# Jittor/PointCloudLib

Measured on AMD Instinct MI355X. Metric: point-clouds/sec fwd+bwd, PointNet++ SSG B=32 N=1024, higher is better.
Workload: dtype f32; 1 GPU; PointNet++ SSG cls train step (fwd+bwd+SGD), B=32/GPU, N=1024 xyz+normal, gauss_ball clouds (BASELINE configs[1]); global_batch=32, n_points=1024, parallelism=dp1, launch=eager, grad_overlap=False, cpu_affinity=numa node 1 (gpu0), 128 cpus, world_size=1, sync_bn=False, entry_points=per-stack (pcl_mlp_stack_*_f32)

## Files before the change

### pointcloudlib_amd/csrc/compact.hip

```cpp
#include "common.h"

namespace pcl {

struct GoffMulti { const int32_t* cnt[4]; int32_t* goff[4]; };
__device__ __forceinline__ void group_offsets_body(const int32_t* __restrict__ cnt, int G, int32_t* __restrict__ goff);
__global__ __launch_bounds__(1024) void group_offsets_kernel(const int32_t* __restrict__ cnt, int G, int32_t* __restrict__ goff) {
    group_offsets_body(cnt, G, goff);
}
__global__ __launch_bounds__(1024) void group_offsets_multi_kernel(const GoffMulti a, int G) {
    group_offsets_body(a.cnt[blockIdx.x], G, a.goff[blockIdx.x]);
}
__device__ __forceinline__ void group_offsets_body(const int32_t* __restrict__ cnt, int G, int32_t* __restrict__ goff) {
    __shared__ int tot[16];
    constexpr int U = 8;
    const int lane = threadIdx.x & 63, w = threadIdx.x >> 6;
    const int per = ((G + 15) / 16 + 63) / 64 * 64;
    const int lo = min(w * per, G), hi = min(lo + per, G);
    int s = 0;
    rows_in_flight<U>(cnt, 1, lo + lane, 64, hi, [&](int, int v) { s += max(v, 1); });
#pragma unroll
    for (int o = 32; o > 0; o >>= 1) s += __shfl_xor(s, o);
    if (lane == 0) tot[w] = s;
    __syncthreads();
    int run = 0, all = 0;
// ... 198 lines not shown
                                                           const int32_t* __restrict__ n_rows, int C1, float* __restrict__ Y,
                                                           double* __restrict__ stats) {
    __shared__ double red[2][4][64 * NH];
    const int wave = threadIdx.x >> 6, lane = threadIdx.x & 63;
    const int R = *n_rows;
    float wx[NH][3], wf[NH][GL_CF];
    double ss[NH], qq[NH];
#pragma unroll
    for (int h = 0; h < NH; ++h) {
        const int ch = lane + 64 * h;
#pragma unroll
        for (int d = 0; d < 3; ++d) wx[h][d] = (Wx && ch < C1) ? Wx[(size_t)ch * ldw + d] : 0.f;
#pragma unroll
        for (int f = 0; f < GL_CF; ++f) wf[h][f] = (f < CF && ch < C1) ? Wfs[(size_t)ch * ldw + f] : 0.f;
        ss[h] = 0.0; qq[h] = 0.0;
    }
    const int stride = gridDim.x * 4 * GL_RPI;
    int r0 = (blockIdx.x * 4 + wave) * GL_RPI;
    float4 nl[GL_RPI], nf[GL_RPI]; int sr[GL_RPI];
#pragma unroll
    for (int j = 0; j < GL_RPI; ++j) {
        const int r = min(r0 + j, R - 1);
        nl[j] = rloc[r]; sr[j] = Uf ? rsrc[r] : 0; nf[j] = CF ? rfeat[r] : make_float4(0.f, 0.f, 0.f, 0.f);
    }
    for (; r0 < R; r0 += stride) {
        float4 L[GL_RPI], F[GL_RPI]; int cs[GL_RPI];
#pragma unroll
        for (int j = 0; j < GL_RPI; ++j) { L[j] = nl[j]; F[j] = nf[j]; cs[j] = sr[j]; }
        {
            const int rn = r0 + stride;
#pragma unroll
            for (int j = 0; j < GL_RPI; ++j) {
                const int r = min(rn + j, R - 1);
                nl[j] = rloc[r]; sr[j] = Uf ? rsrc[r] : 0; nf[j] = CF ? rfeat[r] : make_float4(0.f, 0.f, 0.f, 0.f);
            }
        }
#pragma unroll
        for (int h = 0; h < NH; ++h) {
            const int ch = min(lane + 64 * h, C1 - 1);
            float u[GL_RPI];
#pragma unroll
            for (int j = 0; j < GL_RPI; ++j) u[j] = Uf ? Uf[(size_t)cs[j] * C1 + ch] : 0.f;
#pragma unroll
            for (int j = 0; j < GL_RPI; ++j) {
                if (r0 + j < R && lane + 64 * h < C1) {
                    const float y = glin_row_value(u[j], L[j], F[j], wx[h], wf[h]);
                    Y[(size_t)(r0 + j) * C1 + ch] = y;
                    const double w = (double)L[j].w;
                    ss[h] += w * (double)y; qq[h] += w * (double)y * (double)y;
                }
            }
        }
    }
#pragma unroll
    for (int h = 0; h < NH; ++h) { red[0][wave][lane + 64 * h] = ss[h]; red[1][wave][lane + 64 * h] = qq[h]; }
    __syncthreads();
    for (int ch = threadIdx.x; ch < C1; ch += 256) {
        double* dst = stats + (size_t)blockIdx.x * 2 * C1;
        dst[ch] = (red[0][0][ch] + red[0][1][ch]) + (red[0][2][ch] + red[0][3][ch]);
        dst[C1 + ch] = (red[1][0][ch] + red[1][1][ch]) + (red[1][2][ch] + red[1][3][ch]);
    }
}

template <int NH>
__global__ __launch_bounds__(256) void group_linear_bwd_kernel(const float4* __restrict__ rloc, const float4* __restrict__ rfeat,
                                                               int CF, const float* __restrict__ dU, const float* __restrict__ Y,
                                                               const float* __restrict__ a_, const float* __restrict__ k1_,
                                                               const float* __restrict__ k2_, const float* __restrict__ mu_,
                                                               const int32_t* __restrict__ rsrc,
                                                               const int32_t* __restrict__ n_rows, int C1, float* __restrict__ dUf,
                                                               float* __restrict__ dWx_part, float* __restrict__ dWf_part) {
    __shared__ float red[3 + GL_CF][4][64 * NH];
    const int wave = threadIdx.x >> 6, lane = threadIdx.x & 63;
    const int R = *n_rows;
    float a[NH], k1[NH], k2[NH], mu[NH], gw[NH][3 + GL_CF];
#pragma unroll
    for (int h = 0; h < NH; ++h) {
        const int ch = min(lane + 64 * h, C1 - 1);
        a[h] = a_[ch]; k1[h] = k1_[ch]; k2[h] = k2_[ch]; mu[h] = mu_[ch];
#pragma unroll
        for (int d = 0; d < 3 + GL_CF; ++d) gw[h][d] = 0.f;
    }
    const int stride = gridDim.x * 4 * GL_RPI;
    int r0 = (blockIdx.x * 4 + wave) * GL_RPI;
    float4 nl[GL_RPI], nf[GL_RPI]; int sr[GL_RPI];
#pragma unroll
    for (int j = 0; j < GL_RPI; ++j) {
        const int r = min(r0 + j, R - 1);
        nl[j] = rloc[r]; sr[j] = dUf ? rsrc[r] : 0; nf[j] = dWf_part ? rfeat[r] : make_float4(0.f, 0.f, 0.f, 0.f);
    }
    for (; r0 < R; r0 += stride) {
        float4 L[GL_RPI], F[GL_RPI]; int cs[GL_RPI];
#pragma unroll
        for (int j = 0; j < GL_RPI; ++j) { L[j] = nl[j]; F[j] = nf[j]; cs[j] = sr[j]; }
        {
            const int rn = r0 + stride;
#pragma unroll
            for (int j = 0; j < GL_RPI; ++j) {
                const int r = min(rn + j, R - 1);
                nl[j] = rloc[r]; sr[j] = dUf ? rsrc[r] : 0; nf[j] = dWf_part ? rfeat[r] : make_float4(0.f, 0.f, 0.f, 0.f);
            }
        }
#pragma unroll
        for (int h = 0; h < NH; ++h) {
            const int ch = min(lane + 64 * h, C1 - 1);
            float du[GL_RPI], y[GL_RPI];
#pragma unroll
            for (int j = 0; j < GL_RPI; ++j) {
                const size_t o = (size_t)min(r0 + j, R - 1) * C1 + ch;
                du[j] = dU[o]; y[j] = Y[o];
            }
#pragma unroll
            for (int j = 0; j < GL_RPI; ++j) {
                if (r0 + j < R && lane + 64 * h < C1) {
                    const float dy = fmaf(a[h], du[j], -L[j].w * fmaf(k2[h], y[j] - mu[h], k1[h]));
                    if (dUf) unsafeAtomicAdd(&dUf[(size_t)cs[j] * C1 + ch], dy);
                    gw[h][0] = fmaf(dy, L[j].x, gw[h][0]); gw[h][1] = fmaf(dy, L[j].y, gw[h][1]);
                    gw[h][2] = fmaf(dy, L[j].z, gw[h][2]);
                    gw[h][3] = fmaf(dy, F[j].x, gw[h][3]); gw[h][4] = fmaf(dy, F[j].y, gw[h][4]);
                    gw[h][5] = fmaf(dy, F[j].z, gw[h][5]); gw[h][6] = fmaf(dy, F[j].w, gw[h][6]);
                }
            }
        }
    }
    if (dWx_part || dWf_part) {
#pragma unroll
        for (int h = 0; h < NH; ++h)
#pragma unroll
            for (int d = 0; d < 3 + GL_CF; ++d) red[d][wave][lane + 64 * h] = gw[h][d];
        __syncthreads();
        if (dWx_part)
            for (int e = threadIdx.x; e < C1 * 3; e += 256) {
                const int ch = e / 3, d = e - ch * 3;
                dWx_part[(size_t)blockIdx.x * C1 * 3 + e] = (red[d][0][ch] + red[d][1][ch]) + (red[d][2][ch] + red[d][3][ch]);
            }
        if (dWf_part)
            for (int e = threadIdx.x; e < C1 * CF; e += 256) {
                const int ch = e / CF, d = 3 + (e - ch * CF);
                dWf_part[(size_t)blockIdx.x * C1 * CF + e] = (red[d][0][ch] + red[d][1][ch]) + (red[d][2][ch] + red[d][3][ch]);
            }
    }
}

__device__ __forceinline__ void glin_load_weights(const float* __restrict__ Wx, const float* __restrict__ Wfs, int CF, int ldw, int c4,
                                                  float (&wx)[4][3], float (&wf)[4][GL_CF]) {
#pragma unroll
    for (int v = 0; v < 4; ++v) {
#pragma unroll
        for (int d = 0; d < 3; ++d) wx[v][d] = Wx ? Wx[(size_t)(c4 + v) * ldw + d] : 0.f;
#pragma unroll
        for (int f = 0; f < GL_CF; ++f) wf[v][f] = f < CF ? Wfs[(size_t)(c4 + v) * ldw + f] : 0.f;
    }
}
template <int LPR>
__global__ __launch_bounds__(256) void group_linear_v4_kernel(const float* __restrict__ Uf, const float* __restrict__ Wx,
                                                              const float* __restrict__ Wfs, int CF, int ldw,
                                                              const float4* __restrict__ rloc, const float4* __restrict__ rfeat,
                                                              const int32_t* __restrict__ rsrc,
                                                              const int32_t* __restrict__ n_rows, float* __restrict__ Y,
                                                              double* __restrict__ stats) {
    constexpr int C1 = 4 * LPR, RPW = 64 / LPR, U = 4;
    __shared__ double red[2][4][C1];
    const int wave = threadIdx.x >> 6, lane = threadIdx.x & 63;
    const int cl = lane % LPR, rsub = lane / LPR, c4 = 4 * cl;
    const int R = *n_rows;
    float wx[4][3], wf[4][GL_CF];
    double ss[4], qq[4];
#pragma unroll
    for (int v = 0; v < 4; ++v) {
#pragma unroll
        for (int d = 0; d < 3; ++d) wx[v][d] = Wx ? Wx[(size_t)(c4 + v) * ldw + d] : 0.f;
#pragma unroll
        for (int f = 0; f < GL_CF; ++f) wf[v][f] = f < CF ? Wfs[(size_t)(c4 + v) * ldw + f] : 0.f;
        ss[v] = 0.0; qq[v] = 0.0;
    }
    const int stride = gridDim.x * 4 * RPW * U;
    for (int r0 = (blockIdx.x * 4 + wave) * RPW * U; r0 < R; r0 += stride) {
        float4 L[U], F[U], u[U];
#pragma unroll
        for (int j = 0; j < U; ++j) {
            const int r = min(r0 + j * RPW + rsub, R - 1);
            L[j] = rloc[r];
            F[j] = CF ? rfeat[r] : make_float4(0.f, 0.f, 0.f, 0.f);
            u[j] = Uf ? *reinterpret_cast<const float4*>(Uf + (size_t)rsrc[r] * C1 + c4) : make_float4(0.f, 0.f, 0.f, 0.f);
        }
#pragma unroll
        for (int j = 0; j < U; ++j) {
            const int r = r0 + j * RPW + rsub;
            if (r < R) {
                float y[4] = {u[j].x, u[j].y, u[j].z, u[j].w};
                const double w = (double)L[j].w;
#pragma unroll
                for (int v = 0; v < 4; ++v) {
                    const float t = glin_row_value(y[v], L[j], F[j], wx[v], wf[v]);
                    y[v] = t;
                    ss[v] += w * (double)t; qq[v] += w * (double)t * (double)t;
                }
                *reinterpret_cast<float4*>(Y + (size_t)r * C1 + c4) = make_float4(y[0], y[1], y[2], y[3]);
            }
        }
    }
#pragma unroll
    for (int v = 0; v < 4; ++v) {
#pragma unroll
        for (int off = LPR; off < 64; off <<= 1) { ss[v] += __shfl_xor(ss[v], off); qq[v] += __shfl_xor(qq[v], off); }
        if (rsub == 0) { red[0][wave][c4 + v] = ss[v]; red[1][wave][c4 + v] = qq[v]; }
    }
    __syncthreads();
    for (int ch = threadIdx.x; ch < C1; ch += 256) {
        double* dst = stats + (size_t)blockIdx.x * 2 * C1;
        dst[ch] = (red[0][0][ch] + red[0][1][ch]) + (red[0][2][ch] + red[0][3][ch]);
        dst[C1 + ch] = (red[1][0][ch] + red[1][1][ch]) + (red[1][2][ch] + red[1][3][ch]);
    }
}

template <int LPR>
__global__ __launch_bounds__(256) void group_linear_bwd_v4_kernel(const float4* __restrict__ rloc, const float4* __restrict__ rfeat,
                                                                  int CF, const float* __restrict__ dU, const float* __restrict__ Y,
                                                                  const float* __restrict__ a_, const float* __restrict__ k1_,
                                                                  const float* __restrict__ k2_, const float* __restrict__ mu_,
                                                                  const int32_t* __restrict__ rsrc,
                                                                  const int32_t* __restrict__ n_rows, float* __restrict__ dUf,
                                                                  float* __restrict__ dWx_part, float* __restrict__ dWf_part) {
    constexpr int C1 = 4 * LPR, RPW = 64 / LPR, U = 4;
    __shared__ float red[3 + GL_CF][4][C1];
    const int wave = threadIdx.x >> 6, lane = threadIdx.x & 63;
    const int cl = lane % LPR, rsub = lane / LPR, c4 = 4 * cl;
    const int R = *n_rows;
    float a[4], k1[4], k2[4], mu[4], gw[3 + GL_CF][4];
#pragma unroll
    for (int v = 0; v < 4; ++v) {
        a[v] = a_[c4 + v]; k1[v] = k1_[c4 + v]; k2[v] = k2_[c4 + v]; mu[v] = mu_[c4 + v];
#pragma unroll
        for (int d = 0; d < 3 + GL_CF; ++d) gw[d][v] = 0.f;
    }
    const int stride = gridDim.x * 4 * RPW * U;
    for (int r0 = (blockIdx.x * 4 + wave) * RPW * U; r0 < R; r0 += stride) {
        float4 L[U], F[U], du[U], yv[U];
        int src[U];
#pragma unroll
        for (int j = 0; j < U; ++j) {
            const int r = min(r0 + j * RPW + rsub, R - 1);
            L[j] = rloc[r];
            F[j] = dWf_part ? rfeat[r] : make_float4(0.f, 0.f, 0.f, 0.f);
            src[j] = dUf ? rsrc[r] : 0;
            du[j] = *reinterpret_cast<const float4*>(dU + (size_t)r * C1 + c4);
            yv[j] = *reinterpret_cast<const float4*>(Y + (size_t)r * C1 + c4);
        }
#pragma unroll
        for (int j = 0; j < U; ++j) {
            const int r = r0 + j * RPW + rsub;
            if (r < R) {
                const float dd[4] = {du[j].x, du[j].y, du[j].z, du[j].w}, yy[4] = {yv[j].x, yv[j].y, yv[j].z, yv[j].w};
#pragma unroll
                for (int v = 0; v < 4; ++v) {
                    const float dy = fmaf(a[v], dd[v], -L[j].w * fmaf(k2[v], yy[v] - mu[v], k1[v]));
                    if (dUf) unsafeAtomicAdd(&dUf[(size_t)src[j] * C1 + c4 + v], dy);
                    gw[0][v] = fmaf(dy, L[j].x, gw[0][v]); gw[1][v] = fmaf(dy, L[j].y, gw[1][v]); gw[2][v] = fmaf(dy, L[j].z, gw[2][v]);
                    gw[3][v] = fmaf(dy, F[j].x, gw[3][v]); gw[4][v] = fmaf(dy, F[j].y, gw[4][v]);
                    gw[5][v] = fmaf(dy, F[j].z, gw[5][v]); gw[6][v] = fmaf(dy, F[j].w, gw[6][v]);
                }
            }
        }
    }
    if (dWx_part || dWf_part) {
#pragma unroll
        for (int d = 0; d < 3 + GL_CF; ++d)
#pragma unroll
            for (int v = 0; v < 4; ++v) {
                float t = gw[d][v];
#pragma unroll
                for (int off = LPR; off < 64; off <<= 1) t += __shfl_xor(t, off);
                if (rsub == 0) red[d][wave][c4 + v] = t;
            }
        __syncthreads();
        if (dWx_part)
            for (int e = threadIdx.x; e < C1 * 3; e += 256) {
                const int ch = e / 3, d = e - ch * 3;
                dWx_part[(size_t)blockIdx.x * C1 * 3 + e] = (red[d][0][ch] + red[d][1][ch]) + (red[d][2][ch] + red[d][3][ch]);
            }
        if (dWf_part)
            for (int e = threadIdx.x; e < C1 * CF; e += 256) {
                const int ch = e / CF, d = 3 + (e - ch * CF);
                dWf_part[(size_t)blockIdx.x * C1 * CF + e] = (red[d][0][ch] + red[d][1][ch]) + (red[d][2][ch] + red[d][3][ch]);
            }
    }
}

template <int LPR>
__global__ __launch_bounds__(256) void group_linear_bwd_regen_kernel(const float4* __restrict__ rloc, const float4* __restrict__ rfeat,
                                                                     const float* __restrict__ Wx, const float* __restrict__ Wfs, int CF,
                                                                     int ldw, const float* __restrict__ dU, const float* __restrict__ a_,
                                                                     const float* __restrict__ k1_, const float* __restrict__ k2_,
                                                                     const float* __restrict__ mu_, const int32_t* __restrict__ n_rows,
                                                                     float* __restrict__ dWx_part, float* __restrict__ dWf_part) {
    constexpr int C1 = 4 * LPR, RPW = 64 / LPR, CH = 4, U = 3;
    __shared__ float red[3 + GL_CF][4][C1];
    const int wave = threadIdx.x >> 6, lane = threadIdx.x & 63;
    const int cl = lane % LPR, rsub = lane / LPR, c4 = 4 * cl;
    const int R = *n_rows;
    float wx[4][3], wf[4][GL_CF];
    float a[4], k1[4], k2[4], mu[4], gw[3 + GL_CF][4];
    glin_load_weights(Wx, Wfs, CF, ldw, c4, wx, wf);
#pragma unroll
    for (int v = 0; v < 4; ++v) {
        a[v] = a_[c4 + v]; k1[v] = k1_[c4 + v]; k2[v] = k2_[c4 + v]; mu[v] = mu_[c4 + v];
#pragma unroll
        for (int d = 0; d < 3 + GL_CF; ++d) gw[d][v] = 0.f;
    }
    const int stride = gridDim.x * 4 * RPW * CH, base = (blockIdx.x * 4 + wave) * RPW * CH;
    for (int t0 = 0; base + (t0 / CH) * stride < R; t0 += U) {
        float4 L[U], F[U], du[U];
        int row[U];
#pragma unroll
        for (int j = 0; j < U; ++j) {
            const int t = t0 + j;
            row[j] = base + (t / CH) * stride + (t % CH) * RPW + rsub;
            const int r = min(row[j], R - 1);
            L[j] = rloc[r];
            F[j] = CF ? rfeat[r] : make_float4(0.f, 0.f, 0.f, 0.f);
            du[j] = *reinterpret_cast<const float4*>(dU + (size_t)r * C1 + c4);
        }
#pragma unroll
        for (int j = 0; j < U; ++j) {
            if (row[j] < R) {
                const float dd[4] = {du[j].x, du[j].y, du[j].z, du[j].w};
#pragma unroll
                for (int v = 0; v < 4; ++v) {
                    const float y = glin_row_value(0.f, L[j], F[j], wx[v], wf[v]);
                    const float dy = fmaf(a[v], dd[v], -L[j].w * fmaf(k2[v], y - mu[v], k1[v]));
                    gw[0][v] = fmaf(dy, L[j].x, gw[0][v]); gw[1][v] = fmaf(dy, L[j].y, gw[1][v]); gw[2][v] = fmaf(dy, L[j].z, gw[2][v]);
                    gw[3][v] = fmaf(dy, F[j].x, gw[3][v]); gw[4][v] = fmaf(dy, F[j].y, gw[4][v]);
                    gw[5][v] = fmaf(dy, F[j].z, gw[5][v]); gw[6][v] = fmaf(dy, F[j].w, gw[6][v]);
                }
            }
        }
    }
#pragma unroll
    for (int d = 0; d < 3 + GL_CF; ++d)
#pragma unroll
        for (int v = 0; v < 4; ++v) {
            float t = gw[d][v];
#pragma unroll
            for (int off = LPR; off < 64; off <<= 1) t += __shfl_xor(t, off);
            if (rsub == 0) red[d][wave][c4 + v] = t;
        }
    __syncthreads();
    if (dWx_part)
        for (int e = threadIdx.x; e < C1 * 3; e += 256) {
            const int ch = e / 3, d = e - ch * 3;
            dWx_part[(size_t)blockIdx.x * C1 * 3 + e] = (red[d][0][ch] + red[d][1][ch]) + (red[d][2][ch] + red[d][3][ch]);
        }
// ... 192 lines not shown
    __syncthreads();
    int run = inc - s;
    for (int w = 0; w < wave; ++w) run += wtot[w];
    for (int i = i0; i < i1; ++i) {
        const int t = off[i];
        off[i] = run;
        int pos = run;
        for (int w = 0; w < RT_W; ++w) { const int c = cnt[w * N + i]; cnt[w * N + i] = pos; pos += c; }
        run += t;
    }
    if (tid == 0) off[N] = re - rb;
    __syncthreads();
    for (int g = g0; g < g1; ++g) {
        const int q0 = group_off[g_first + g], q1 = group_off[g_first + g + 1];
        for (int r = q0 + lane; r < q1; r += 64) lst[atomicAdd(&mycnt[rsrc[r] - pbase], 1)] = r;
        __builtin_amdgcn_fence(__ATOMIC_SEQ_CST, "wavefront");
        __builtin_amdgcn_wave_barrier();
    }
    __syncthreads();
    for (int pl = tid; pl < N; pl += RT_T) in_off[pbase + pl] = rb + off[pl];
    if (b == B - 1 && tid == 0) in_off[pbase + N] = re;
    for (int i = tid; i < re - rb; i += RT_T) in_rows[rb + i] = lst[i];
}

__global__ __launch_bounds__(256) void group_linear_dw_kernel(const float* __restrict__ px, const float* __restrict__ pf, int rows,
                                                              int C1, int CF, int off, int ld, float* __restrict__ dW0) {
    const int nx = px ? C1 * 3 : 0, nf = pf ? C1 * CF : 0;
    const int e = blockIdx.x * 4 + (threadIdx.x >> 6), lane = threadIdx.x & 63;
    if (e >= nx + nf) return;
    const bool isx = e < nx;
    const float* src = isx ? px + e : pf + (e - nx);
    const int n = isx ? nx : nf;
    float s = 0.f;
    rows_in_flight<8>(src, n, lane, 64, rows, [&](int, float v) { s += v; });
#pragma unroll
    for (int o = 32; o > 0; o >>= 1) s += __shfl_xor(s, o);
    if (lane == 0) {
        if (isx) dW0[(size_t)(e / 3) * ld + e % 3] = s;
        else dW0[(size_t)((e - nx) / CF) * ld + off + (e - nx) % CF] = s;
    }
}

}
using namespace pcl;

extern "C" int pcl_group_offsets_i32(const int32_t* cnt, int G, int32_t* group_off, void* stream) {
    PCL_REQUIRE(cnt && group_off && G >= 1, "pcl_group_offsets_i32: bad arguments");
    hipLaunchKernelGGL(group_offsets_kernel, dim3(1), dim3(1024), 0, as_stream(stream), cnt, G, group_off);
    return check_launch("pcl_group_offsets_i32");
}

extern "C" int pcl_group_offsets_multi_i32(int n, const int32_t* const* cnt, int G, int32_t* const* group_off, void* stream) {
    PCL_REQUIRE(cnt && group_off && G >= 1 && n >= 1 && n <= 4, "pcl_group_offsets_multi_i32: bad arguments (n = %d: 1..4)", n);
    GoffMulti a = {};
    for (int i = 0; i < n; ++i) {
        PCL_REQUIRE(cnt[i] && group_off[i], "pcl_group_offsets_multi_i32: null array %d", i);
        a.cnt[i] = cnt[i]; a.goff[i] = group_off[i];
    }
    hipLaunchKernelGGL(group_offsets_multi_kernel, dim3(n), dim3(1024), 0, as_stream(stream), a, G);
    return check_launch("pcl_group_offsets_multi_i32");
}

extern "C" int pcl_group_compact_f32(const float* xyz, const float* new_xyz, const float* feat, const int32_t* idx,
                                     const int32_t* cnt, const int32_t* group_off, int B, int N, int m, int ns, int C,
                                     int use_xyz, int row_stride, float* rows, int32_t* row_meta, int32_t* row_src,
                                     void* stream) {
    PCL_REQUIRE(idx && cnt && rows && row_meta && row_src && group_off, "pcl_group_compact_f32: null pointer");
    PCL_REQUIRE(!use_xyz || (xyz && new_xyz), "pcl_group_compact_f32: use_xyz needs xyz and new_xyz");
    PCL_REQUIRE(C == 0 || feat, "pcl_group_compact_f32: C=%d needs feat", C);
    PCL_REQUIRE(B >= 1 && N >= 1 && m >= 1 && ns >= 1 && ns < 32768 && C >= 0 && (use_xyz || C > 0), "pcl_group_compact_f32: bad sizes");
    const int D = (use_xyz ? 3 : 0) + C;
    PCL_REQUIRE(row_stride >= D && row_stride < D + 64, "pcl_group_compact_f32: row_stride=%d for %d columns", row_stride, D);
    const int G = B * m;
    hipLaunchKernelGGL(group_compact_kernel, dim3(G), dim3(256), 0, as_stream(stream), xyz, new_xyz, feat, idx, cnt, group_off, G, N, m,
                       ns, C, use_xyz, row_stride, rows, reinterpret_cast<int2*>(row_meta), row_src);
    return check_launch("pcl_group_compact_f32");
}

extern "C" int pcl_bn_act_max_rows_f32(const float* Y, const int32_t* group_off, const float* scale, const float* shift,
                                       float slope, int G, int C, float* out, int32_t* arg, float* ymax, void* stream) {
    PCL_REQUIRE(Y && group_off && scale && shift && out && arg && ymax && G >= 1 && C >= 1, "pcl_bn_act_max_rows_f32: bad arguments");
    const bool vec = (C % 4 == 0) && al16(Y);
    const size_t total = (size_t)G * (vec ? C / 4 : C);
    int blocks = (int)((total + 255) / 256);
    if (blocks > 16384) blocks = 16384;
    if (vec)
        hipLaunchKernelGGL(bn_act_max_rows_kernel<4>, dim3(blocks), dim3(256), 0, as_stream(stream), Y, group_off, scale, shift, slope,
                           G, C, out, arg, ymax);
    else
        hipLaunchKernelGGL(bn_act_max_rows_kernel<1>, dim3(blocks), dim3(256), 0, as_stream(stream), Y, group_off, scale, shift, slope,
                           G, C, out, arg, ymax);
    return check_launch("pcl_bn_act_max_rows_f32");
}

extern "C" int pcl_scatter_rows_add_f32(const float* grows, const int32_t* row_src, const int32_t* n_rows_dev, int rows_cap,
                                        int D, int off, int C, int n_dst_rows, float* gfeat, void* stream) {
    PCL_REQUIRE(grows && row_src && n_rows_dev && gfeat && rows_cap >= 1 && D >= 1 && off >= 0 && C >= 1 && off + C <= D && n_dst_rows >= 1,
                "pcl_scatter_rows_add_f32: bad arguments");
    hipStream_t st = as_stream(stream);
    hipError_t e = hipMemsetAsync(gfeat, 0, sizeof(float) * (size_t)n_dst_rows * C, st);
    if (e != hipSuccess) return fail(PCL_EHIP, "pcl_scatter_rows_add_f32: memset: %s", hipGetErrorString(e));
    size_t blocks = ((size_t)rows_cap + 7) / 8;
    if (blocks > 8192) blocks = 8192;
    hipLaunchKernelGGL(scatter_rows_add_kernel, dim3((int)blocks), dim3(256), 0, st, grows, row_src, n_rows_dev, D, off, C, gfeat);
    return check_launch("pcl_scatter_rows_add_f32");
}

constexpr int GL_BLOCKS = 1024;

extern "C" int pcl_group_linear_stat_rows(int B, int m) { return (B < 1 || m < 1) ? 0 : GL_BLOCKS; }

namespace pcl {
int group_linear_fwd_impl(const float* xyz, const float* new_xyz, const float* Uf, const float* Wx, const float* feat_small,
                          const float* Wf_small, int CF, int ldw, const int32_t* idx, const int32_t* cnt, const int32_t* group_off, int B,
                          int N, int m, int ns, int C1, float* Y, int32_t* row_meta, int32_t* row_src, float* row_loc, float* row_feat,
                          double* stats_ws, void* stream, int phase, const float* dense_src, float* dense_dst, int dense_cols);
}
extern "C" int pcl_group_linear_f32(const float* xyz, const float* new_xyz, const float* Uf, const float* Wx, const float* feat_small,
                                    const float* Wf_small, int CF, int ldw, const int32_t* idx, const int32_t* cnt,
                                    const int32_t* group_off, int B, int N, int m, int ns, int C1, float* Y, int32_t* row_meta,
                                    int32_t* row_src, float* row_loc, float* row_feat, double* stats_ws, void* stream) {
    return group_linear_fwd_impl(xyz, new_xyz, Uf, Wx, feat_small, Wf_small, CF, ldw, idx, cnt, group_off, B, N, m, ns, C1, Y, row_meta, row_src,
                                 row_loc, row_feat, stats_ws, stream, 3, nullptr, nullptr, 0);
}
int pcl::group_linear_fwd_impl(const float* xyz, const float* new_xyz, const float* Uf, const float* Wx, const float* feat_small,
                               const float* Wf_small, int CF, int ldw, const int32_t* idx, const int32_t* cnt, const int32_t* group_off,
                               int B, int N, int m, int ns, int C1, float* Y, int32_t* row_meta, int32_t* row_src, float* row_loc,
                               float* row_feat, double* stats_ws, void* stream, int phase, const float* dense_src, float* dense_dst,
                               int dense_cols) {
    PCL_REQUIRE(idx && cnt && group_off && Y && row_meta && row_src && row_loc && stats_ws, "pcl_group_linear_f32: null pointer");
    PCL_REQUIRE(CF == 0 || row_feat, "pcl_group_linear_f32: inline features need row_feat");
    PCL_REQUIRE(phase == 1 || Uf || Wx || CF > 0, "pcl_group_linear_f32: need features (Uf or feat_small) and/or coordinates (Wx)");
    PCL_REQUIRE(CF >= 0 && CF <= GL_CF && (CF == 0 || (feat_small && Wf_small)), "pcl_group_linear_f32: CF=%d inline features (<= %d)", CF, GL_CF);
    PCL_REQUIRE(!Wx || (xyz && new_xyz), "pcl_group_linear_f32: Wx needs xyz and new_xyz");
    PCL_REQUIRE(ldw >= (Wx ? 3 : 0) && ldw >= CF, "pcl_group_linear_f32: ldw=%d", ldw);
    PCL_REQUIRE(B >= 1 && N >= 1 && m >= 1 && ns >= 1 && ns < 32768 && C1 >= 1 && C1 <= 64 * GL_MAXH,
                "pcl_group_linear_f32: bad sizes B=%d N=%d m=%d ns=%d C1=%d (C1 <= %d)", B, N, m, ns, C1, 64 * GL_MAXH);
    const int G = B * m;
    hipStream_t st = as_stream(stream);
    if (phase & 1) {
        const int gb = (G + 3) / 4;
        DenseJob dj = {dense_src, dense_dst, C1, dense_cols, ldw, gb, 0};
        if (dense_dst) dj.blocks = (C1 * dense_cols + 1023) / 1024 < 64 ? (C1 * dense_cols + 1023) / 1024 : 64;
        hipLaunchKernelGGL(group_rows_meta_kernel, dim3(gb + dj.blocks), dim3(256), 0, st, Wx ? xyz : nullptr, new_xyz, feat_small, CF, idx, cnt,
                           group_off, G, N, m, ns, reinterpret_cast<int2*>(row_meta), row_src, reinterpret_cast<float4*>(row_loc),
                           reinterpret_cast<float4*>(CF ? row_feat : nullptr), dj);
        int rc = check_launch("pcl_group_linear_f32(meta)");
        if (rc || phase == 1) return rc;
    }
    const float4* rl = reinterpret_cast<const float4*>(row_loc);
    const float4* rf = reinterpret_cast<const float4*>(row_feat);
    const dim3 grid(GL_BLOCKS), block(256);
    if (al16(Y, Uf) && (C1 == 64 || C1 == 128 || C1 == 256)) {
        if (C1 == 64) hipLaunchKernelGGL(group_linear_v4_kernel<16>, grid, block, 0, st, Uf, Wx, Wf_small, CF, ldw, rl, rf, row_src, group_off + G, Y, stats_ws);
        else if (C1 == 128) hipLaunchKernelGGL(group_linear_v4_kernel<32>, grid, block, 0, st, Uf, Wx, Wf_small, CF, ldw, rl, rf, row_src, group_off + G, Y, stats_ws);
        else hipLaunchKernelGGL(group_linear_v4_kernel<64>, grid, block, 0, st, Uf, Wx, Wf_small, CF, ldw, rl, rf, row_src, group_off + G, Y, stats_ws);
        return check_launch("pcl_group_linear_f32");
    }
    if (C1 <= 64) hipLaunchKernelGGL(group_linear_kernel<1>, grid, block, 0, st, Uf, Wx, Wf_small, CF, ldw, rl, rf, row_src, group_off + G, C1, Y, stats_ws);
    else if (C1 <= 128) hipLaunchKernelGGL(group_linear_kernel<2>, grid, block, 0, st, Uf, Wx, Wf_small, CF, ldw, rl, rf, row_src, group_off + G, C1, Y, stats_ws);
    else hipLaunchKernelGGL(group_linear_kernel<4>, grid, block, 0, st, Uf, Wx, Wf_small, CF, ldw, rl, rf, row_src, group_off + G, C1, Y, stats_ws);
    return check_launch("pcl_group_linear_f32");
}

namespace pcl {
int group_linear_bwd_impl(const float* row_loc, const float* row_feat, int CF, const float* dU, const float* Y, const float* a,
                          const float* k1, const float* k2, const float* mu, const int32_t* row_src, const int32_t* n_rows_dev, int B, int N,
                          int C1, float* dUf, float* dWx_part, float* dWf_part, float* dW0, int ldw, int off, void* stream, bool duf_is_zero);
}
extern "C" int pcl_group_linear_bwd_f32(const float* row_loc, const float* row_feat, int CF, const float* dU, const float* Y,
                                        const float* a, const float* k1, const float* k2, const float* mu, const int32_t* row_src,
                                        const int32_t* n_rows_dev, int B, int N, int C1, float* dUf, float* dWx_part,
                                        float* dWf_part, float* dW0, int ldw, int off, void* stream) {
    return group_linear_bwd_impl(row_loc, row_feat, CF, dU, Y, a, k1, k2, mu, row_src, n_rows_dev, B, N, C1, dUf, dWx_part, dWf_part, dW0, ldw,
                                 off, stream, false);
}
int pcl::group_linear_bwd_impl(const float* row_loc, const float* row_feat, int CF, const float* dU, const float* Y, const float* a,
                               const float* k1, const float* k2, const float* mu, const int32_t* row_src, const int32_t* n_rows_dev, int B,
                               int N, int C1, float* dUf, float* dWx_part, float* dWf_part, float* dW0, int ldw, int off, void* stream,
                               bool duf_is_zero) {
    PCL_REQUIRE(row_loc && dU && Y && a && k1 && k2 && mu && row_src && n_rows_dev, "pcl_group_linear_bwd_f32: null pointer");
    PCL_REQUIRE(dUf || dWx_part || dWf_part, "pcl_group_linear_bwd_f32: nothing to compute");
    PCL_REQUIRE(!dWf_part || (row_feat && CF >= 1 && CF <= GL_CF), "pcl_group_linear_bwd_f32: dWf needs row_feat, CF=%d", CF);
    PCL_REQUIRE(B >= 1 && N >= 1 && C1 >= 1 && C1 <= 64 * GL_MAXH, "pcl_group_linear_bwd_f32: bad sizes");
    PCL_REQUIRE(!dW0 || ((dWx_part || dWf_part) && ldw >= (dWx_part ? 3 : 0) && off >= 0 && ldw >= off + (dWf_part ? CF : 0)),
                "pcl_group_linear_bwd_f32: dW0 needs the partial buffers and ldw=%d >= off=%d + CF", ldw, off);
    hipStream_t st = as_stream(stream);
    if (dUf && !duf_is_zero) {
        hipError_t e = hipMemsetAsync(dUf, 0, sizeof(float) * (size_t)B * N * C1, st);
        if (e != hipSuccess) return fail(PCL_EHIP, "pcl_group_linear_bwd_f32: memset: %s", hipGetErrorString(e));
    }
    const float4* rl = reinterpret_cast<const float4*>(row_loc);
    const float4* rf = reinterpret_cast<const float4*>(row_feat);
    const dim3 grid(GL_BLOCKS), block(256);
    if (!dUf && al16(Y, dU) && (C1 == 64 || C1 == 128 || C1 == 256)) {
        if (C1 == 64) hipLaunchKernelGGL(group_linear_bwd_v4_kernel<16>, grid, block, 0, st, rl, rf, CF, dU, Y, a, k1, k2, mu, row_src, n_rows_dev, dUf, dWx_part, dWf_part);
        else if (C1 == 128) hipLaunchKernelGGL(group_linear_bwd_v4_kernel<32>, grid, block, 0, st, rl, rf, CF, dU, Y, a, k1, k2, mu, row_src, n_rows_dev, dUf, dWx_part, dWf_part);
        else hipLaunchKernelGGL(group_linear_bwd_v4_kernel<64>, grid, block, 0, st, rl, rf, CF, dU, Y, a, k1, k2, mu, row_src, n_rows_dev, dUf, dWx_part, dWf_part);
    } else if (C1 <= 64) hipLaunchKernelGGL(group_linear_bwd_kernel<1>, grid, block, 0, st, rl, rf, CF, dU, Y, a, k1, k2, mu, row_src, n_rows_dev, C1, dUf, dWx_part, dWf_part);
    else if (C1 <= 128) hipLaunchKernelGGL(group_linear_bwd_kernel<2>, grid, block, 0, st, rl, rf, CF, dU, Y, a, k1, k2, mu, row_src, n_rows_dev, C1, dUf, dWx_part, dWf_part);
    else hipLaunchKernelGGL(group_linear_bwd_kernel<4>, grid, block, 0, st, rl, rf, CF, dU, Y, a, k1, k2, mu, row_src, n_rows_dev, C1, dUf, dWx_part, dWf_part);
    int rc = check_launch("pcl_group_linear_bwd_f32");
    if (rc || !dW0) return rc;
    const int n = (dWx_part ? C1 * 3 : 0) + (dWf_part ? C1 * CF : 0);
    hipLaunchKernelGGL(group_linear_dw_kernel, dim3((n + 3) / 4), block, 0, st, dWx_part, dWf_part, GL_BLOCKS, C1, CF, off, ldw, dW0);
    return check_launch("pcl_group_linear_bwd_f32(dW)");
}

extern "C" int pcl_group_linear_dw_sum_f32(const float* dWx_part, const float* dWf_part, int rows, int C1, int CF, int off, int ld, float* dW0,
                                           void* stream) {
    PCL_REQUIRE((dWx_part || dWf_part) && dW0 && rows >= 1 && C1 >= 1, "pcl_group_linear_dw_sum_f32: bad arguments");
    PCL_REQUIRE(!dWf_part || CF >= 1, "pcl_group_linear_dw_sum_f32: dWf_part needs CF >= 1");
    PCL_REQUIRE(ld >= (dWx_part ? 3 : 0) && off >= 0 && ld >= off + (dWf_part ? CF : 0), "pcl_group_linear_dw_sum_f32: ld=%d below off=%d + CF", ld, off);
    const int n = (dWx_part ? C1 * 3 : 0) + (dWf_part ? C1 * CF : 0);
    hipLaunchKernelGGL(group_linear_dw_kernel, dim3((n + 3) / 4), dim3(256), 0, as_stream(stream), dWx_part, dWf_part, rows, C1, CF, off, ld, dW0);
    return check_launch("pcl_group_linear_dw_sum_f32");
}

extern "C" int pcl_group_rows_transpose_supported(int N, int m, int ns) {
    return N >= 1 && m >= 1 && ns >= 1 && ((size_t)(RT_W + 1) * N + 1 + (size_t)m * ns) * 4 <= 150 * 1024;
}
extern "C" int pcl_group_rows_transpose_i32(const int32_t* row_src, const int32_t* group_off, int B, int N, int m, int ns, int32_t* in_off,
                                            int32_t* in_rows, void* stream) {
    PCL_REQUIRE(row_src && group_off && in_off && in_rows && B >= 1 && m >= 1 && ns >= 1, "pcl_group_rows_transpose_i32: bad arguments");
    PCL_REQUIRE(pcl_group_rows_transpose_supported(N, m, ns), "pcl_group_rows_transpose_i32: N=%d m=%d ns=%d beyond the LDS-resident form", N, m, ns);
    const size_t lds = ((size_t)(RT_W + 1) * N + 1 + (size_t)m * ns) * 4;
    auto kern = rows_transpose_kernel;
    if (int rc = lds_opt_in(kern, lds, "pcl_group_rows_transpose_i32")) return rc;
    hipLaunchKernelGGL(kern, dim3(B), dim3(RT_T), lds, as_stream(stream), row_src, group_off, m, N, B, in_off, in_rows);
    return check_launch("pcl_group_rows_transpose_i32");
}
extern "C" int pcl_group_linear_bwd_gather_supported(int C1) { return g_lab.scatter_gather && (C1 == 64 || C1 == 128 || C1 == 256); }
extern "C" int pcl_group_linear_bwd_gather_f32(const float* row_loc, const float* dU, const float* Y, const float* a, const float* k1,
                                               const float* k2, const float* mu, const int32_t* in_off, const int32_t* in_rows, int B, int N,
                                               int C1, float* dUf, float* dWx_part, float* dW0, int ldw, void* stream) {
    PCL_REQUIRE(row_loc && dU && Y && a && k1 && k2 && mu && in_off && in_rows && dUf, "pcl_group_linear_bwd_gather_f32: null pointer");
    PCL_REQUIRE(B >= 1 && N >= 1 && pcl_group_linear_bwd_gather_supported(C1), "pcl_group_linear_bwd_gather_f32: bad sizes (C1 = %d: 64, 128 or 256)", C1);
    PCL_REQUIRE(al16(dU, Y, dUf) && al16(a, k1, k2, mu), "pcl_group_linear_bwd_gather_f32: 16-byte aligned rows");
    PCL_REQUIRE(!dW0 || (dWx_part && ldw >= 3), "pcl_group_linear_bwd_gather_f32: dW0 needs dWx_part and ldw >= 3");
    hipStream_t st = as_stream(stream);
    const float4* rl = reinterpret_cast<const float4*>(row_loc);
    const dim3 grid(GL_BLOCKS), block(256);
    const int P = B * N;
    if (C1 == 64) hipLaunchKernelGGL(group_linear_bwd_gather_kernel<16>, grid, block, 0, st, rl, dU, Y, a, k1, k2, mu, in_off, in_rows, P, dUf, dWx_part);
    else if (C1 == 128) hipLaunchKernelGGL(group_linear_bwd_gather_kernel<32>, grid, block, 0, st, rl, dU, Y, a, k1, k2, mu, in_off, in_rows, P, dUf, dWx_part);
    else hipLaunchKernelGGL(group_linear_bwd_gather_kernel<64>, grid, block, 0, st, rl, dU, Y, a, k1, k2, mu, in_off, in_rows, P, dUf, dWx_part);
    int rc = check_launch("pcl_group_linear_bwd_gather_f32");
    if (rc || !dW0) return rc;
    hipLaunchKernelGGL(group_linear_dw_kernel, dim3((C1 * 3 + 3) / 4), block, 0, st, dWx_part, (const float*)nullptr, GL_BLOCKS, C1, 0, 0, ldw, dW0);
    return check_launch("pcl_group_linear_bwd_gather_f32(dW)");
}

extern "C" int pcl_group_linear_bwd_regen_supported(int C1, int CF) {
    return (C1 == 64 || C1 == 128 || C1 == 256) && CF >= 0 && CF <= GL_CF;
}
extern "C" int pcl_group_linear_bwd_regen_f32(const float* row_loc, const float* row_feat, const float* Wx, const float* Wf_small, int CF,
                                              int ldw, const float* dU, const float* a, const float* k1, const float* k2, const float* mu,
                                              const int32_t* n_rows_dev, int C1, float* dWx_part, float* dWf_part, float* dW0, int ld0, int off,
                                              void* stream) {
    PCL_REQUIRE(row_loc && dU && a && k1 && k2 && mu && n_rows_dev, "pcl_group_linear_bwd_regen_f32: null pointer");
    PCL_REQUIRE(pcl_group_linear_bwd_regen_supported(C1, CF), "pcl_group_linear_bwd_regen_f32: C1 = %d (64, 128 or 256), CF = %d (<= %d)", C1, CF, GL_CF);
    PCL_REQUIRE(Wx || CF > 0, "pcl_group_linear_bwd_regen_f32: need the forward's weights (Wx and/or Wf_small)");
    PCL_REQUIRE(CF == 0 || (row_feat && Wf_small), "pcl_group_linear_bwd_regen_f32: CF=%d inline features need row_feat and Wf_small", CF);
    PCL_REQUIRE(ldw >= (Wx ? 3 : 0) && ldw >= CF, "pcl_group_linear_bwd_regen_f32: ldw=%d", ldw);
    PCL_REQUIRE(dWx_part || dWf_part, "pcl_group_linear_bwd_regen_f32: nothing to compute");
    PCL_REQUIRE(!dWf_part || CF >= 1, "pcl_group_linear_bwd_regen_f32: dWf_part needs CF >= 1");
    PCL_REQUIRE(al16(dU, row_loc, row_feat), "pcl_group_linear_bwd_regen_f32: 16-byte aligned rows");
    PCL_REQUIRE(!dW0 || (ld0 >= (dWx_part ? 3 : 0) && off >= 0 && ld0 >= off + (dWf_part ? CF : 0)),
                "pcl_group_linear_bwd_regen_f32: dW0 needs ld0=%d >= off=%d + CF", ld0, off);
    hipStream_t st = as_stream(stream);
    const float4* rl = reinterpret_cast<const float4*>(row_loc);
    const float4* rf = reinterpret_cast<const float4*>(row_feat);
    const dim3 grid(GL_BLOCKS), block(256);
    if (C1 == 64) hipLaunchKernelGGL(group_linear_bwd_regen_kernel<16>, grid, block, 0, st, rl, rf, Wx, Wf_small, CF, ldw, dU, a, k1, k2, mu, n_rows_dev, dWx_part, dWf_part);
    else if (C1 == 128) hipLaunchKernelGGL(group_linear_bwd_regen_kernel<32>, grid, block, 0, st, rl, rf, Wx, Wf_small, CF, ldw, dU, a, k1, k2, mu, n_rows_dev, dWx_part, dWf_part);
    else hipLaunchKernelGGL(group_linear_bwd_regen_kernel<64>, grid, block, 0, st, rl, rf, Wx, Wf_small, CF, ldw, dU, a, k1, k2, mu, n_rows_dev, dWx_part, dWf_part);
    int rc = check_launch("pcl_group_linear_bwd_regen_f32");
    if (rc || !dW0) return rc;
    const int n = (dWx_part ? C1 * 3 : 0) + (dWf_part ? C1 * CF : 0);
    hipLaunchKernelGGL(group_linear_dw_kernel, dim3((n + 3) / 4), block, 0, st, dWx_part, dWf_part, GL_BLOCKS, C1, CF, off, ld0, dW0);
    return check_launch("pcl_group_linear_bwd_regen_f32(dW)");
}
extern "C" int pcl_group_linear_bwd_gather_regen_f32(const float* row_loc, const float* dU, const float* Uf, const float* Wx, int ldw,
                                                     const float* a, const float* k1, const float* k2, const float* mu, const int32_t* in_off,
                                                     const int32_t* in_rows, int B, int N, int C1, float* dUf, float* dWx_part, float* dW0,
                                                     int ld0, void* stream) {
    PCL_REQUIRE(row_loc && dU && Uf && a && k1 && k2 && mu && in_off && in_rows && dUf, "pcl_group_linear_bwd_gather_regen_f32: null pointer");
    PCL_REQUIRE(B >= 1 && N >= 1 && pcl_group_linear_bwd_gather_supported(C1), "pcl_group_linear_bwd_gather_regen_f32: bad sizes (C1 = %d: 64, 128 or 256)", C1);
    PCL_REQUIRE(al16(dU, Uf, dUf, row_loc) && al16(a, k1, k2, mu), "pcl_group_linear_bwd_gather_regen_f32: 16-byte aligned rows");
    PCL_REQUIRE(!Wx || ldw >= 3, "pcl_group_linear_bwd_gather_regen_f32: ldw=%d", ldw);
    PCL_REQUIRE(!dW0 || (dWx_part && ld0 >= 3), "pcl_group_linear_bwd_gather_regen_f32: dW0 needs dWx_part and ld0 >= 3");
    hipStream_t st = as_stream(stream);
    const float4* rl = reinterpret_cast<const float4*>(row_loc);
    const dim3 grid(GL_BLOCKS), block(256);
    const int P = B * N;
    if (C1 == 64) hipLaunchKernelGGL(group_linear_bwd_gather_regen_kernel<16>, grid, block, 0, st, rl, dU, Uf, Wx, ldw, a, k1, k2, mu, in_off, in_rows, P, dUf, dWx_part);
    else if (C1 == 128) hipLaunchKernelGGL(group_linear_bwd_gather_regen_kernel<32>, grid, block, 0, st, rl, dU, Uf, Wx, ldw, a, k1, k2, mu, in_off, in_rows, P, dUf, dWx_part);
    else hipLaunchKernelGGL(group_linear_bwd_gather_regen_kernel<64>, grid, block, 0, st, rl, dU, Uf, Wx, ldw, a, k1, k2, mu, in_off, in_rows, P, dUf, dWx_part);
    int rc = check_launch("pcl_group_linear_bwd_gather_regen_f32");
    if (rc || !dW0) return rc;
    hipLaunchKernelGGL(group_linear_dw_kernel, dim3((C1 * 3 + 3) / 4), block, 0, st, dWx_part, (const float*)nullptr, GL_BLOCKS, C1, 0, 0, ld0, dW0);
    return check_launch("pcl_group_linear_bwd_gather_regen_f32(dW)");
}
```

Before: 18090 point-clouds/s.

## Software-pipeline group_linear_v4 loads and specialize kernel on input presence

Rewrites the forward group-linear v4 kernel main loop as a two-half double-buffered pipeline. Loads for the next half (row loc/feat, gathered Uf rows and the next source indices) are issued before the current half is computed, with sched_barrier and asm register pinning to keep the compiler from reordering them. The kernel is also templated on whether Uf, Wx and features are present, so the per-row null checks disappear. This is meant to hide gather latency, at the cost of more register pressure, more template instantiations and a separate tail path.

Result: no change. 18220 point-clouds/s, median of 4 (+0.7%).

```diff
diff --git a/pointcloudlib_amd/csrc/compact.hip b/pointcloudlib_amd/csrc/compact.hip
--- a/pointcloudlib_amd/csrc/compact.hip
+++ b/pointcloudlib_amd/csrc/compact.hip
@@ -374,7 +374,11 @@
         for (int f = 0; f < GL_CF; ++f) wf[v][f] = f < CF ? Wfs[(size_t)(c4 + v) * ldw + f] : 0.f;
     }
 }
-template <int LPR>
+
+template <bool HU, bool HF>
+struct GlinHalf { float4 L[2], F[HF ? 2 : 1], u[HU ? 2 : 1]; };
+
+template <int LPR, bool HU, bool HX, bool HF>
 __global__ __launch_bounds__(256) void group_linear_v4_kernel(const float* __restrict__ Uf, const float* __restrict__ Wx,
                                                               const float* __restrict__ Wfs, int CF, int ldw,
                                                               const float4* __restrict__ rloc, const float4* __restrict__ rfeat,
@@ -383,7 +387,7 @@
                                                               double* __restrict__ stats) {
     constexpr int C1 = 4 * LPR, RPW = 64 / LPR, U = 4;
     __shared__ double red[2][4][C1];
-    const int wave = threadIdx.x >> 6, lane = threadIdx.x & 63;
+    const int wave = __builtin_amdgcn_readfirstlane(threadIdx.x >> 6), lane = threadIdx.x & 63;
     const int cl = lane % LPR, rsub = lane / LPR, c4 = 4 * cl;
     const int R = *n_rows;
     float wx[4][3], wf[4][GL_CF];
@@ -391,35 +395,80 @@
 #pragma unroll
     for (int v = 0; v < 4; ++v) {
 #pragma unroll
-        for (int d = 0; d < 3; ++d) wx[v][d] = Wx ? Wx[(size_t)(c4 + v) * ldw + d] : 0.f;
-#pragma unroll
-        for (int f = 0; f < GL_CF; ++f) wf[v][f] = f < CF ? Wfs[(size_t)(c4 + v) * ldw + f] : 0.f;
+        for (int d = 0; d < 3; ++d) { wx[v][d] = 0.f; if constexpr (HX) wx[v][d] = Wx[(size_t)(c4 + v) * ldw + d]; }
+#pragma unroll
+        for (int f = 0; f < GL_CF; ++f) {
+            wf[v][f] = 0.f;
+            if constexpr (HF) { const float t = Wfs[(size_t)(c4 + v) * ldw + min(f, CF - 1)]; wf[v][f] = f < CF ? t : 0.f; }
+        }
         ss[v] = 0.0; qq[v] = 0.0;
     }
+    using Half = GlinHalf<HU, HF>;
     const int stride = gridDim.x * 4 * RPW * U;
-    for (int r0 = (blockIdx.x * 4 + wave) * RPW * U; r0 < R; r0 += stride) {
-        float4 L[U], F[U], u[U];
-#pragma unroll
-        for (int j = 0; j < U; ++j) {
-            const int r = min(r0 + j * RPW + rsub, R - 1);
-            L[j] = rloc[r];
-            F[j] = CF ? rfeat[r] : make_float4(0.f, 0.f, 0.f, 0.f);
-            u[j] = Uf ? *reinterpret_cast<const float4*>(Uf + (size_t)rsrc[r] * C1 + c4) : make_float4(0.f, 0.f, 0.f, 0.f);
-        }
-#pragma unroll
-        for (int j = 0; j < U; ++j) {
-            const int r = r0 + j * RPW + rsub;
-            if (r < R) {
-                float y[4] = {u[j].x, u[j].y, u[j].z, u[j].w};
-                const double w = (double)L[j].w;
-#pragma unroll
-                for (int v = 0; v < 4; ++v) {
-                    const float t = glin_row_value(y[v], L[j], F[j], wx[v], wf[v]);
-                    y[v] = t;
-                    ss[v] += w * (double)t; qq[v] += w * (double)t * (double)t;
-                }
-                *reinterpret_cast<float4*>(Y + (size_t)r * C1 + c4) = make_float4(y[0], y[1], y[2], y[3]);
-            }
+    int r0 = (blockIdx.x * 4 + wave) * RPW * U;
+    int sn[2];
+    auto row_at = [&](auto* rec, int base, int j) {
+        const int sb = min(base, R - 1);
+        return rec[sb + (unsigned)min(j * RPW + rsub, R - 1 - sb)];
+    };
+    auto request_src = [&](int base, int j0) {
+#pragma unroll
+        for (int i = 0; i < 2; ++i) sn[i] = row_at(rsrc, base, j0 + i);
+    };
+    auto request = [&](Half& o, int base, int j0, int nbase, int nj0) {
+#pragma unroll
+        for (int i = 0; i < 2; ++i) {
+            o.L[i] = row_at(rloc, base, j0 + i);
+            if constexpr (HF) o.F[i] = row_at(rfeat, base, j0 + i);
+        }
+        if constexpr (HU) {
+#pragma unroll
+            for (int i = 0; i < 2; ++i) o.u[i] = *reinterpret_cast<const float4*>(Uf + (size_t)sn[i] * C1 + c4);
+            request_src(nbase, nj0);
+        }
+        __builtin_amdgcn_sched_barrier(0);
+    };
+    auto arrive = [&](Half& o) {
+        __builtin_amdgcn_sched_barrier(0);
+#pragma unroll
+        for (int i = 0; i < 2; ++i) {
+            asm volatile("" : "+v"(o.L[i].x), "+v"(o.L[i].y), "+v"(o.L[i].z), "+v"(o.L[i].w));
+            if constexpr (HF) asm volatile("" : "+v"(o.F[i].x), "+v"(o.F[i].y), "+v"(o.F[i].z), "+v"(o.F[i].w));
+            if constexpr (HU) asm volatile("" : "+v"(o.u[i].x), "+v"(o.u[i].y), "+v"(o.u[i].z), "+v"(o.u[i].w), "+v"(sn[i]));
+        }
+    };
+    auto row_values = [&](const Half& o, int j) {
+        const float4 z = make_float4(0.f, 0.f, 0.f, 0.f);
+        const float4 L = o.L[j & 1], F = HF ? o.F[j & 1] : z, u = HU ? o.u[j & 1] : z;
+        float y[4] = {u.x, u.y, u.z, u.w};
+        const double w = (double)L.w;
+#pragma unroll
+        for (int v = 0; v < 4; ++v) {
+            const float t = glin_row_value(y[v], L, F, wx[v], wf[v]);
+            y[v] = t;
+            ss[v] += w * (double)t; qq[v] += w * (double)t * (double)t;
+        }
+        *reinterpret_cast<float4*>(Y + (size_t)r0 * C1 + (unsigned)((j * RPW + rsub) * C1 + c4)) = make_float4(y[0], y[1], y[2], y[3]);
+    };
+    if (r0 < R) {
+        Half P, Q;
+        if constexpr (HU) request_src(r0, 0);
+        request(P, r0, 0, r0, 2);
+        arrive(P);
+        for (; r0 + U * RPW <= R; r0 += stride) {
+            request(Q, r0, 2, r0 + stride, 0);
+            row_values(P, 0); row_values(P, 1);
+            arrive(Q);
+            request(P, r0 + stride, 0, r0 + stride, 2);
+            row_values(Q, 2); row_values(Q, 3);
+            arrive(P);
+        }
+        if (r0 < R) {
+            request(Q, r0, 2, r0, 2);
+            arrive(Q);
+#pragma unroll
+            for (int j = 0; j < U; ++j)
+                if (r0 + j * RPW + rsub < R) row_values(j < 2 ? P : Q, j);
         }
     }
 #pragma unroll
@@ -918,9 +967,25 @@
     const float4* rf = reinterpret_cast<const float4*>(row_feat);
     const dim3 grid(GL_BLOCKS), block(256);
     if (al16(Y, Uf) && (C1 == 64 || C1 == 128 || C1 == 256)) {
-        if (C1 == 64) hipLaunchKernelGGL(group_linear_v4_kernel<16>, grid, block, 0, st, Uf, Wx, Wf_small, CF, ldw, rl, rf, row_src, group_off + G, Y, stats_ws);
-        else if (C1 == 128) hipLaunchKernelGGL(group_linear_v4_kernel<32>, grid, block, 0, st, Uf, Wx, Wf_small, CF, ldw, rl, rf, row_src, group_off + G, Y, stats_ws);
-        else hipLaunchKernelGGL(group_linear_v4_kernel<64>, grid, block, 0, st, Uf, Wx, Wf_small, CF, ldw, rl, rf, row_src, group_off + G, Y, stats_ws);
+        auto launch = [&](auto lpr) {
+            auto with = [&](auto hu, auto hx, auto hf) {
+                hipLaunchKernelGGL((group_linear_v4_kernel<decltype(lpr)::value, decltype(hu)::value, decltype(hx)::value, decltype(hf)::value>), grid, block, 0, st, Uf, Wx, Wf_small, CF, ldw, rl, rf, row_src,
+                                   group_off + G, Y, stats_ws);
+            };
+            const std::true_type yes; const std::false_type no;
+            switch ((Uf ? 4 : 0) | (Wx ? 2 : 0) | (CF ? 1 : 0)) {
+                case 1: with(no, no, yes); break;
+                case 2: with(no, yes, no); break;
+                case 3: with(no, yes, yes); break;
+                case 4: with(yes, no, no); break;
+                case 5: with(yes, no, yes); break;
+                case 6: with(yes, yes, no); break;
+                default: with(yes, yes, yes); break;
+            }
+        };
+        if (C1 == 64) launch(std::integral_constant<int, 16>());
+        else if (C1 == 128) launch(std::integral_constant<int, 32>());
+        else launch(std::integral_constant<int, 64>());
         return check_launch("pcl_group_linear_f32");
     }
     if (C1 <= 64) hipLaunchKernelGGL(group_linear_kernel<1>, grid, block, 0, st, Uf, Wx, Wf_small, CF, ldw, rl, rf, row_src, group_off + G, C1, Y, stats_ws);
```
